# junwenxiong/diff_sal

Measured on AMD Instinct MI355X. Metric: denoise-steps/sec (batch x NFE / wall time), 16x224x384 clip, 50-step DPM-Solver, higher is better.
Workload: dtype f32; 1 GPU; BASELINE configs[1]: DHF1k visual-only, batch=4/GPU, 224x384, 50-NFE DPM-Solver (multistep-2, logSNR, denoise-to-zero), faithful full graph; batch_per_gpu=4, nfe_per_trajectory=50, step=one SalUNet evaluation + DPM-Solver update on one batch, sampler_mode=eager

## Files before the change

diff_sal_amd/_lib.py:

```python
import ctypes as C
import os

from . import build as _build

_LIB = None

c_f = C.c_void_p
c_i = C.c_int
c_fl = C.c_float
c_sz = C.c_size_t


class ConvDesc(C.Structure):

    _fields_ = [(n, C.c_int) for n in (
        "N", "H", "W", "Cin", "Ho", "Wo", "Cout", "KH", "KW", "stride_h", "stride_w", "pad_t", "pad_l",
        "dil_h", "dil_w", "act", "rowvec_ld", "w_format", "precision", "dtype")]


class Wino4Ext(C.Structure):

    _fields_ = [("in_ab", C.c_void_p), ("side_a", C.c_void_p), ("side_w", C.c_void_p), ("side_out", C.c_void_p),
                ("out_stats", C.c_void_p), ("up2_c", C.c_void_p), ("up2_scale", C.c_void_p), ("up2_shift", C.c_void_p),
                ("side_rows", C.c_longlong), ("in_swish", C.c_int), ("out_groups", C.c_int), ("up2_act", C.c_int), ("reserved", C.c_int)]


ABI_VERSION = 43


SIGNATURES = {
    "diffsal_version": (c_i, []),
    "diffsal_last_error": (C.c_char_p, []),
    "diffsal_last_gemm_kernel": (C.c_char_p, []),
    "diffsal_conv_igemm_group": (c_i, [c_i, c_f, c_f, c_f, c_f, c_f, c_f, c_sz, c_f]),
    "diffsal_kv_prep_proj": (c_i, [c_f] * 14 + [c_i, c_i, c_i, c_i, c_i, c_fl, c_f, c_f, c_fl, c_i, c_i, c_f]),
    "diffsal_block_front": (c_i, [c_f, c_f, c_f, c_f, c_f, c_fl, c_f, c_f, c_f, c_fl, c_f, c_f, c_f, c_f, c_f, c_i, c_i, c_i, c_i,
                                  c_i, c_i, c_fl, c_i, c_f]),
    "diffsal_set_tuning": (c_i, [C.c_char_p, c_i]),
    "diffsal_get_tuning": (c_i, [C.c_char_p]),
    "diffsal_temb_mlp": (c_i, [c_f, c_i, c_i, c_i, c_f, c_f, c_f, c_f, c_f, c_f, c_f, c_f]),
    "diffsal_dense_small": (c_i, [c_f, c_i, c_i, c_i, c_f, c_f, c_i, c_f, c_f]),
    "diffsal_conv_in": (c_i, [c_f, c_f, c_f, c_f, c_i, c_i, c_i, c_i, c_i, c_i, c_i, c_f]),
    "diffsal_maxpool2d": (c_i, [c_f, c_f, c_i, c_i, c_i, c_i, c_i, c_i, c_i, c_f]),
    "diffsal_conv_in_s4": (c_i, [c_f, c_f, c_f, c_f, c_i, c_i, c_i, c_i, c_i, c_f]),
    "diffsal_tapsum": (c_i, [c_f, c_f, c_f, c_i, c_f, c_i, c_i, c_i, c_i, c_i, c_f, c_f, c_f, c_i, c_i, c_f]),
    "diffsal_tapsum_head": (c_i, [c_f, c_f, c_f, c_i, c_i, c_i, c_i, c_i, c_i, c_f, c_f, c_f, c_i, c_f, c_f, c_f, c_i, c_f]),
    "diffsal_tapsum_bwd_ws_bytes": (C.c_long, [c_i, c_i, c_i, c_i]),
    "diffsal_tapsum_bwd": (c_i, [c_f, c_f, c_f, c_i, c_i, c_i, c_i, c_i, c_i, c_i, c_f]),
    "diffsal_groupnorm_ws_bytes": (c_sz, [c_i, c_i]),
    "diffsal_groupnorm_swish": (c_i, [c_f, c_f, c_f, c_f, c_i, c_i, c_i, c_i, c_fl, c_f, c_sz, c_i, c_f]),
    "diffsal_groupnorm": (c_i, [c_f, c_f, c_f, c_f, c_i, c_i, c_i, c_i, c_fl, c_i, c_f, c_sz, c_i, c_f]),
    "diffsal_softmax_rows": (c_i, [c_f, c_f, C.c_long, c_i, c_fl, c_f]),
# ... 176 lines not shown
```

diff_sal_amd/csrc/common.h:

```cpp
#pragma once
#include <hip/hip_runtime.h>

#include <cstdarg>
#include <cstdint>
#include <cstdio>

#include "../../include/diffsal.h"

namespace diffsal {

void set_error(const char* fmt, ...);
void note_kernel(const char* fmt, ...);

inline bool aligned16(const void* p) { return (reinterpret_cast<uintptr_t>(p) & 15u) == 0; }

inline int check_launch(const char* what) {
  hipError_t e = hipGetLastError();
  if (e != hipSuccess) {
    set_error("%s: launch failed: %s", what, hipGetErrorString(e));
    return DIFFSAL_E_LAUNCH;
  }
  return DIFFSAL_OK;
}

#define DS_REQUIRE(cond, code, ...)  \
  do {                               \
    if (!(cond)) {                   \
      diffsal::set_error(__VA_ARGS__); \
      return (code);                 \
    }                                \
  } while (0)

constexpr int kWave = 64;

enum TuneKey {
  TUNE_NO_PERSIST = 0, TUNE_NO_XCD_ORDER, TUNE_NO_HALO, TUNE_FORCE_HALO, TUNE_IGEMM_CFG, TUNE_IGEMM16_CFG, TUNE_PLAN_DEBUG,
  TUNE_WGRAD_CFG, TUNE_WGRAD_SPLITS, TUNE_WGRAD_VERBOSE, TUNE_NO_FUSED_BLOCK, TUNE_NO_WINOGRAD, TUNE_FORCE_WINOGRAD, TUNE_GN_CHUNKS,
  TUNE_GN_APPLY_WGS, TUNE_GEMM_DMA, TUNE_CONV_DMA, TUNE_GROUP_GRID, TUNE_GEMM_DMA16, TUNE_WGRAD_DMA, TUNE_NO_GN_SLAB, TUNE_NO_WINOGRAD4, TUNE_BATCH_TILE, TUNE_BATCH_XCD, TUNE_NO_TAPSUM_ROWS, TUNE_TAPSUM_ROWS_FORM,
  TUNE_NO_ATTN_BWD_DS, TUNE_NO_POOL_RUNS, TUNE_NO_ATTN_SLOTS, TUNE_NO_STREAM16, TUNE_CONV16_TILE, TUNE_BLOCK16_WAVES, TUNE_NO_ATTN16_MFMA, TUNE_CONV16_HALF, TUNE_COUNT
};
int tune(int key);

template <int CTRL>
__device__ __forceinline__ float dpp_move(float v) {
  return __builtin_bit_cast(float, __builtin_amdgcn_update_dpp(0, __builtin_bit_cast(int, v), CTRL, 0xF, 0xF, false));
}
__device__ __forceinline__ float lane_xor16(float v) {
  const unsigned u = __builtin_bit_cast(unsigned, v);
  const auto r = __builtin_amdgcn_permlane16_swap(u, u, false, false);
  return __builtin_bit_cast(float, (__lane_id() & 16) ? r[0] : r[1]);
}
__device__ __forceinline__ float lane_xor32(float v) {
  const unsigned u = __builtin_bit_cast(unsigned, v);
  const auto r = __builtin_amdgcn_permlane32_swap(u, u, false, false);
// ... 290 lines not shown
```

diff_sal_amd/csrc/misc.hip:

```cpp
#include "common.h"

#include <cstdlib>
#include <cstring>

namespace diffsal {

static thread_local char g_err[512] = "";
void set_error(const char* fmt, ...) {
  va_list ap;
  va_start(ap, fmt);
  vsnprintf(g_err, sizeof(g_err), fmt, ap);
  va_end(ap);
}

static thread_local char g_kernel[160] = "";
void note_kernel(const char* fmt, ...) {
  va_list ap;
  va_start(ap, fmt);
  vsnprintf(g_kernel, sizeof(g_kernel), fmt, ap);
  va_end(ap);
}

static const char* const kTuneNames[TUNE_COUNT] = {
    "DIFFSAL_NO_PERSIST", "DIFFSAL_NO_XCD_ORDER", "DIFFSAL_NO_HALO", "DIFFSAL_FORCE_HALO", "DIFFSAL_IGEMM_CFG",
    "DIFFSAL_IGEMM16_CFG", "DIFFSAL_PLAN_DEBUG", "DIFFSAL_WGRAD_CFG", "DIFFSAL_WGRAD_SPLITS", "DIFFSAL_WGRAD_VERBOSE",
    "DIFFSAL_NO_FUSED_BLOCK", "DIFFSAL_NO_WINOGRAD", "DIFFSAL_FORCE_WINOGRAD", "DIFFSAL_GN_CHUNKS", "DIFFSAL_GN_APPLY_WGS",
    "DIFFSAL_GEMM_DMA", "DIFFSAL_CONV_DMA", "DIFFSAL_GROUP_GRID", "DIFFSAL_GEMM_DMA16", "DIFFSAL_WGRAD_DMA", "DIFFSAL_NO_GN_SLAB", "DIFFSAL_NO_WINOGRAD4", "DIFFSAL_BATCH_TILE", "DIFFSAL_BATCH_XCD", "DIFFSAL_NO_TAPSUM_ROWS", "DIFFSAL_TAPSUM_ROWS_FORM",
    "DIFFSAL_NO_ATTN_BWD_DS", "DIFFSAL_NO_POOL_RUNS", "DIFFSAL_NO_ATTN_SLOTS", "DIFFSAL_NO_STREAM16", "DIFFSAL_CONV16_TILE", "DIFFSAL_BLOCK16_WAVES", "DIFFSAL_NO_ATTN16_MFMA", "DIFFSAL_CONV16_HALF"};
static int g_tune[TUNE_COUNT];
static const bool g_tune_init = [] {
  for (int k = 0; k < TUNE_COUNT; ++k) {
    const char* e = getenv(kTuneNames[k]);
    g_tune[k] = (e && e[0]) ? atoi(e) : -1;
  }
  return true;
}();
int tune(int key) { return (key >= 0 && key < TUNE_COUNT) ? __atomic_load_n(&g_tune[key], __ATOMIC_RELAXED) : -1; }

__global__ __launch_bounds__(256) void temb_dense0_kernel(const void* __restrict__ t, int t_is_f32, int B, int ch,
                                                          const float* __restrict__ freq, const float* __restrict__ w0,
                                                          const float* __restrict__ b0, float* __restrict__ hid) {
  extern __shared__ float sh[];
  const int half = ch / 2, tc = 4 * ch;
// ... 849 lines not shown
    case DIFFSAL_WS_CONV_WINO4_STATS: return d && have && n_dims == 1 ? diffsal_conv_wino4_stats_bytes(d, D(0)) : 0;
    case DIFFSAL_WS_CONV_WGRAD: return d ? diffsal_conv_wgrad_ws_bytes(d) : 0;
    case DIFFSAL_WS_WGRAD_SEGMENTED: return have && n_dims == 4 ? diffsal_wgrad_segmented_ws_bytes(D(0), D(1), D(2), D(3)) : 0;
    case DIFFSAL_WS_TAPSUM_BWD: return have && n_dims == 4 ? static_cast<size_t>(diffsal_tapsum_bwd_ws_bytes(D(0), D(1), D(2), D(3))) : 0;
    case DIFFSAL_WS_SALIENCY_METRICS: return have && n_dims == 1 ? diffsal_saliency_metrics_ws_bytes(D(0)) : 0;
    case DIFFSAL_WS_ATTENTION_TAIL:
      return have && n_dims == 5 ? sizeof(float) * diffsal_attention_general_tail_floats(D(0), D(1), D(2), D(3), D(4)) : 0;
    case DIFFSAL_WS_ATTENTION_BWD_QTAIL:
      return have && n_dims == 6 ? sizeof(float) * diffsal_attention_general_bwd_qtail_floats(D(0), D(1), D(2), D(3), D(4), D(5)) : 0;
    case DIFFSAL_WS_ATTENTION_BWD_DS:
      return have && n_dims == 4 ? sizeof(float) * diffsal_attention_general_bwd_ds_floats(D(0), D(1), D(2), D(3)) : 0;
    default: return 0;
  }
}

extern "C" int diffsal_version(void) { return 43; }
extern "C" const char* diffsal_last_error(void) { return g_err; }
extern "C" const char* diffsal_last_gemm_kernel(void) { return g_kernel; }

extern "C" int diffsal_set_tuning(const char* name, int value) {
  DS_REQUIRE(name, DIFFSAL_E_ARG, "set_tuning: null name");
  for (int k = 0; k < TUNE_COUNT; ++k)
    if (strcmp(name, kTuneNames[k]) == 0) {
      __atomic_store_n(&g_tune[k], value, __ATOMIC_RELAXED);
      return DIFFSAL_OK;
    }
  set_error("set_tuning: unknown switch '%s'", name);
  return DIFFSAL_E_ARG;
}
extern "C" int diffsal_get_tuning(const char* name) {
  if (name)
// ... 550 lines not shown
```

diff_sal_amd/csrc/tblock.hip:

```cpp
#include "common.h"

namespace diffsal {

template <> struct Mfma32x16<float> { typedef f32x8_t vec; };

template <typename T>
struct FrontArgs {
  const T* x;
  const T* k;
  const T* v;
  const float* g1; const float* b1;
  const float* w9;
  const float* gq; const float* bq;
  const T* wq; const float* bias_q;
  const T* wp; const float* bias_p;
  T* out;
  int N, H, W, Lk;
  float eps1, epsq, scale;
  int tiles_y, tiles_x;
#ifdef DIFFSAL_DEV_STAMPS
  unsigned long long* stamps;
#endif
};

// ... 487 lines not shown
template <typename T, int C>
static int launch_front(const FrontArgs<T>& a, hipStream_t s) {
  typedef FrontLds<T, C> L;
  DS_RAISE_DYNAMIC_LDS((block_front_kernel<T, C>), 160 * 1024);
  const int n_tiles = a.N * a.tiles_y * a.tiles_x;
  const int resident = 256 * (L::total * 2 <= 160 * 1024 ? 2 : 1);
  const int grid = n_tiles < resident ? n_tiles : resident;
#ifdef DIFFSAL_DEV_STAMPS
  FrontArgs<T> b = a;
  b.stamps = (g_front_stamps && static_cast<size_t>(grid) * 64 * 8 <= g_front_stamp_bytes) ? g_front_stamps : nullptr;
  hipLaunchKernelGGL((block_front_kernel<T, C>), dim3(grid), dim3(256), L::total, s, b);
  return check_launch("block_front");
#endif
  hipLaunchKernelGGL((block_front_kernel<T, C>), dim3(grid), dim3(256), L::total, s, a);
  return check_launch("block_front");
}

}

using namespace diffsal;

#ifdef DIFFSAL_DEV_STAMPS
extern "C" int diffsal_set_front_stamps(void* device_buffer, size_t bytes) {
  diffsal::g_front_stamps = static_cast<unsigned long long*>(device_buffer);
  diffsal::g_front_stamp_bytes = device_buffer ? bytes : 0;
  return DIFFSAL_OK;
}
#endif

extern "C" int diffsal_block_front(const void* x, const void* k, const void* v, const float* g1, const float* b1, float eps1,
// ... 18 lines not shown
  {                                                                                                                         \
    FrontArgs<T> a{static_cast<const T*>(x), static_cast<const T*>(k), static_cast<const T*>(v), g1, b1, w9, gq, bq,        \
                   static_cast<const T*>(wq), bias_q, static_cast<const T*>(wp), bias_p, static_cast<T*>(out), N, H, W, Lk, \
                   eps1, epsq, scale, tiles_y, tiles_x};                                                                    \
    return launch_front<T, CC>(a, s);                                                                                       \
  }
  if (dtype == DIFFSAL_F32) DS_FRONT(float, 96)
  if (C == 96) {
    if (dtype == DIFFSAL_BF16) DS_FRONT(bf16_t, 96)
    DS_FRONT(f16_t, 96)
  }
  if (dtype == DIFFSAL_BF16) DS_FRONT(bf16_t, 192)
  DS_FRONT(f16_t, 192)
#undef DS_FRONT
}
```

diff_sal_amd/ops.py:

```python
from __future__ import annotations

import contextlib
import ctypes as C
import threading
from typing import List, Optional, Sequence, Tuple

import torch

from . import _lib
from ._lib import ACT_GELU, ACT_GELU_GRAD, ACT_NONE, ACT_RELU, ACT_SIGMOID, ConvDesc

Tensor = torch.Tensor

PROFILE = None


_PROF_DEPTH = [0]


class _prof:
    __slots__ = ("cls", "flops", "nbytes", "e0", "note", "counted", "kernel")

    def __init__(self, cls, flops=0.0, nbytes=0.0, note="", kernel=""):
        self.cls, self.flops, self.nbytes, self.e0, self.note, self.counted = cls, float(flops), float(nbytes), None, note, False
# ... 965 lines not shown
    with_p = x.dtype == torch.float32
    if with_p and lin_p is None:
        raise RuntimeError("block_front: fp32 storage needs the output projection")
    M = N * H * W
    fl = 2.0 * M * Cc * Cc * (2 if with_p else 1) + 4.0 * M * Lk * Cc + 22.0 * M * Cc
    with _prof("K10f", fl, _nb(x, out, k, v, lin_q[0]) + (_nb(lin_p[0]) if with_p else 0.0), f"block_front M={M} C={Cc}",
               kernel=f"block_front_kernel<{'float' if with_p else '16-bit'}, {Cc}>"):
        _lib.check(lib.diffsal_block_front(_pa(x, dt), _pa(k, dt), _pa(v, dt), _p(norm1[0]), _p(norm1[1]), float(norm1[2]),
                                           _p(w9), _p(norm_q[0]), _p(norm_q[1]), float(norm_q[2]), _pa(lin_q[0], dt),
                                           _p(lin_q[1]), _pa(lin_p[0], dt) if with_p else None,
                                           _p(lin_p[1]) if with_p else None, out.data_ptr(), N, H, W, Cc, Lk, heads,
                                           float(scale), dt, _stream()), "block_front")
    return out


def dwpool_ln_kv(xk: Tensor, xv: Tensor, wk: Tensor, wv: Tensor, gk: Tensor, bk: Tensor, gv: Tensor, bv: Tensor,
                 k: int, eps: float = 1e-5):
    lib = _lib.load()
    N, H, W, Cc = xv.shape
    gh, gw = (H - k) // k + 1, (W - k) // k + 1
    ok = torch.empty((N, gh * gw, Cc), device=xv.device, dtype=xv.dtype)
    ov = torch.empty_like(ok)
    dt = _dt(xv)
    with _prof("K9", 4.0 * N * H * W * Cc, _nb(xk, ok, ov) + (0.0 if xk.data_ptr() == xv.data_ptr() else _nb(xv))):
        _lib.check(lib.diffsal_dwpool_ln_kv(_pa(xk, dt), _pa(xv, dt), _p(wk), _p(wv), _p(gk), _p(bk), _p(gv), _p(bv),
                                            ok.data_ptr(), ov.data_ptr(), N, H, W, Cc, k, eps, dt, _stream()), "dwpool_ln_kv")
    return ok, ov


def attention(q: Tensor, k: Tensor, v: Tensor, heads: int, scale: float) -> Tensor:
# ... 890 lines not shown
```

diff_sal_amd/sal_unet.py:

```python
from __future__ import annotations

import math
from typing import Dict, List, Optional, Sequence

import torch
from torch import nn

from . import ops
from .ops import ACT_GELU, ACT_NONE, ACT_RELU

Tensor = torch.Tensor


def _holder(**children) -> nn.Module:
    m = nn.Module()
    for k, v in children.items():
        setattr(m, k, v)
    return m


def _seq_named(pairs) -> nn.Sequential:
    from collections import OrderedDict

    return nn.Sequential(OrderedDict(pairs))
# ... 163 lines not shown
                if m.bias is not None:
                    nn.init.zeros_(m.bias)
            elif isinstance(m, (nn.LayerNorm, nn.BatchNorm2d, nn.GroupNorm)):
                nn.init.ones_(m.weight)
                nn.init.zeros_(m.bias)
        for st in self.invpt_decoder.mid_stages:
            for m in st.modules():
                if isinstance(m, nn.Linear):
                    nn.init.trunc_normal_(m.weight, std=0.02)
        nn.init.trunc_normal_(self.invpt_decoder.mt_proj[0].weight, std=0.02)

    def _precision(self) -> str:
        return self.gemm_precision or ops.get_gemm_precision()

    def _cache_key(self):
        return (self._pack_epoch, self._precision(), self.compute_dtype, self.winograd, self.fold_attn_proj) + tuple(
            (p.data_ptr(), p._version) for p in list(self.parameters()) + list(self.buffers()))

    def pack_epoch(self):
        return self._cache_key()

    def parameters_updated(self) -> None:
        self._pack_epoch += 1

    def _pack_conv(self, w: Tensor) -> Tensor:
        wp = ops.pack_conv_weight(w)
        if self.compute_dtype != torch.float32:
            return ops.cast(wp, self.compute_dtype)
        return ops.split_weight(wp) if self._precision() == "bf16x3" else wp

    def _pack_wino(self, w: Tensor, f2: bool = True):
# ... 8 lines not shown
    def _use_tap_conv(self, taps, which: str) -> bool:
        if not self.tap_conv or (taps is not None and self.taps_reference_forms):
            return False
        if (which == "mt" and self.compute_dtype != torch.float32 and self.mt_tap16_f32 and self.fold_head
                and self.ori_embed_dim % 192 == 0):
            return True
        return self.compute_dtype == torch.float32 or which in self.tap_conv16

    def _gemm_w(self, w: Tensor) -> Tensor:
        return w.detach() if self.compute_dtype == torch.float32 else ops.cast(w.detach().contiguous(), self.compute_dtype)

    def _fold_attn(self, i: int, Lk: int) -> bool:
        return (self.fold_attn_proj and self.compute_dtype == torch.float32 and self._precision() == "fp32"
                and ops.attn_fold_supported(self.up_channels[i], self.heads[i], Lk, torch.float32))

    @staticmethod
    def fold_attn_weights(a: nn.Module):
        c = a.proj_q.weight.shape[0]
        d = c // 2
        wq, wk, wv, wp = (l.weight.detach().double() for l in (a.proj_q, a.proj_k, a.proj_v, a.proj))
        zero = wq.new_zeros(c)
        bq, bv, bp = ((l.bias.detach().double() if l.bias is not None else zero) for l in (a.proj_q, a.proj_v, a.proj))
        kq, vp, ukq = [], [], []
        for h in range(2):
            s = slice(h * d, (h + 1) * d)
            kq.append(wq[s].t() @ wk[s])
            vp.append(wp[:, s] @ wv[s])
            ukq.append(wk[s].t() @ bq[s])
        return (torch.cat(kq, 0).float().contiguous(), torch.cat(vp, 0).float().contiguous(),
                torch.stack(ukq, 0).float().contiguous(), (bp + wp @ bv).float().contiguous())

    @staticmethod
    def _bn_affine(bn: nn.BatchNorm2d):
        scale = (bn.weight.detach() / torch.sqrt(bn.running_var + bn.eps)).contiguous()
        shift = (bn.bias.detach() - bn.running_mean * scale).contiguous()
        return scale, shift

    def packed(self) -> Dict[str, Tensor]:
        key = self._cache_key()
        if self._pack_cache is not None and key == self._pack_key:
            return self._pack_cache
        dev = self.conv_in.weight.device
        pk: Dict[str, Tensor] = {}
        half = self.ch // 2
        pk["freq"] = torch.exp(torch.arange(half, dtype=torch.float32) * -(math.log(10000) / (half - 1))).to(dev)
# ... 28 lines not shown
                pk[f"s{i}.pe2.w"] = self._pack_conv(pe[4].weight)
                pk[f"s{i}.pe2.wino"] = self._pack_wino(pe[4].weight)
                pk[f"s{i}.pe2.scale"], pk[f"s{i}.pe2.shift"] = self._bn_affine(pe[5])
            a = st.blocks[0].attn
            c = self.up_channels[i]
            k = self.kernel_kv[i]
            pk[f"s{i}.wq9"] = a.conv_proj_q.conv.weight.detach()[:, 0, 1].reshape(c, 9).t().contiguous()
            pk[f"s{i}.wk"] = a.conv_proj_k.conv.weight.detach().reshape(c, k * k).t().contiguous()
            pk[f"s{i}.wv"] = a.conv_proj_v.conv.weight.detach().reshape(c, k * k).t().contiguous()
            pk[f"s{i}.align.w"] = self._gemm_w(st.blocks[0].align_conv.weight.detach().reshape(c, 512).contiguous())
            blk = st.blocks[0]
            for nm, lin in (("q", a.proj_q), ("k", a.proj_k), ("v", a.proj_v), ("proj", a.proj), ("fc1", blk.mlp.fc1),
                            ("fc2", blk.mlp.fc2)):
                pk[f"s{i}.{nm}.w"] = self._gemm_w(lin.weight)
            pk[f"s{i}.redu.w"] = self._pack_conv(dec.redu_chan_up[i].proj[0].weight)
            if self._fold_attn(i, 1):
                pk[f"s{i}.kq.w"], pk[f"s{i}.vp.w"], pk[f"s{i}.ukq"], pk[f"s{i}.proj.bf"] = self.fold_attn_weights(a)
        if all(f"s{i}.align.w" in pk for i in range(self.num_stages)) and self.num_stages > 1:
            pk["align_all.w"] = torch.cat([pk[f"s{i}.align.w"] for i in range(self.num_stages)], 0).contiguous()
            pk["align_all.b"] = torch.cat([dec.mid_stages[i].blocks[0].align_conv.bias.detach().float()
                                           for i in range(self.num_stages)], 0).contiguous()
            offs, o = [], 0
            for i in range(self.num_stages):
                offs.append(o)
                o += self.up_channels[i]
            pk["align_all.offs"] = offs
        pk["mt.w"] = self._pack_conv(dec.mt_proj[0].weight)
        pk["mt.tapw"] = self._tap_weight(dec.mt_proj[0].weight)
        pk["mt.scale"], pk["mt.shift"] = self._bn_affine(dec.mt_proj[1])
        pk["head.w"] = self.logits.linear_pred.weight.detach().reshape(-1).contiguous()
        self._pack_cache, self._pack_key = pk, key
# ... 74 lines not shown
            if isinstance(audio_tok, tuple):
                a_all, offs = audio_tok
                a_small = a_all[:, :, offs[i]:offs[i] + C]
            else:
                a_small = ops.linear(audio_tok, pk[f"s{i}.align.w"], blk.align_conv.bias, tag="K7-align")
            k_src = ops.audio_fuse(a_small, x, audio_hw[0], audio_hw[1])
        xt = x.view(n9, H * W, C)
        gh, gw = (H - self.kernel_kv[i]) // self.kernel_kv[i] + 1, (W - self.kernel_kv[i]) // self.kernel_kv[i] + 1
        if (self.fused_front and ops.block_front_supported(C, self.heads[i], gh * gw, x.dtype)
                and (x.dtype != torch.float32 or self._precision() == "fp32")
                and not getattr(pk[f"s{i}.k.w"], "_diffsal_split", False)):
            xv_ = x.view(n9, H, W, C)
            xk_ = xv_ if k_src is None else k_src.view(n9, H, W, C)
            kvn = (a.conv_proj_k.bn.weight, a.conv_proj_k.bn.bias, a.conv_proj_v.bn.weight, a.conv_proj_v.bn.bias)
            pre = (blk.norm.weight, blk.norm.bias, blk.norm.eps, k_src is None)
            if self.fold_kv_proj and C == 96:
                kk, vv = ops.kv_prep_proj(xk_, xv_, pk[f"s{i}.wk"], pk[f"s{i}.wv"], *kvn, self.kernel_kv[i], a.conv_proj_k.bn.eps, pre,
                                          (pk[f"s{i}.k.w"], a.proj_k.bias), (pk[f"s{i}.v.w"], a.proj_v.bias))
            else:
                kk, vv = ops.kv_prep(xk_, xv_, pk[f"s{i}.wk"], pk[f"s{i}.wv"], *kvn, self.kernel_kv[i], a.conv_proj_k.bn.eps, pre_ln=pre)
                kk, vv = ops.linear_pair(kk, vv, pk[f"s{i}.k.w"], pk[f"s{i}.v.w"], a.proj_k.bias, a.proj_v.bias)
            f32 = x.dtype == torch.float32
            y = ops.block_front(xv_, kk, vv, (blk.norm.weight, blk.norm.bias, blk.norm.eps), pk[f"s{i}.wq9"],
                                (a.conv_proj_q.bn.weight, a.conv_proj_q.bn.bias, a.conv_proj_q.bn.eps),
                                (pk[f"s{i}.q.w"], a.proj_q.bias), (pk[f"s{i}.proj.w"], a.proj.bias) if f32 else None,
                                self.heads[i], float(C) ** -0.5).view(n9, H * W, C)
            nz = None if norm_z is None else (norm_z.weight, norm_z.bias, norm_z.eps)
            if C == 96 and blk.mlp.fc1.out_features == 192:
                if f32:
                    x2, z = ops.mlp_block(y, (blk.norm2.weight, blk.norm2.bias, blk.norm2.eps), (pk[f"s{i}.fc1.w"], blk.mlp.fc1.bias),
                                          (pk[f"s{i}.fc2.w"], blk.mlp.fc2.bias), nz, (H * W, T, self.temporal_list[i]))
                else:
                    x2, z = ops.block16(y, xt, (pk[f"s{i}.proj.w"], a.proj.bias), (blk.norm2.weight, blk.norm2.bias, blk.norm2.eps),
                                        (pk[f"s{i}.fc1.w"], blk.mlp.fc1.bias), (pk[f"s{i}.fc2.w"], blk.mlp.fc2.bias), nz,
                                        (H * W, T, self.temporal_list[i]))
                return x2.view(B, T, H, W, C), (None if z is None else z.view(B, T, H, W, C))
            x1 = y if f32 else ops.linear(y, pk[f"s{i}.proj.w"], a.proj.bias, residual=xt)
            y2 = ops.layernorm(x1, blk.norm2.weight, blk.norm2.bias, blk.norm2.eps)
            y2 = ops.linear(y2, pk[f"s{i}.fc1.w"], blk.mlp.fc1.bias, act=ACT_GELU)
            x2 = ops.linear(y2, pk[f"s{i}.fc2.w"], blk.mlp.fc2.bias, residual=x1)
            return x2.view(B, T, H, W, C), None
# ... 73 lines not shown
                    per_clip.append(T * h * w * 9 * self.up_channels[i])
                h, w = 2 * h, 2 * w
            per_clip.append(T * h * w * self.up_channels[i] * 2)
            tok += h * w
        per_clip.append(tok * 9 * self.down_channel * (2 if es == 2 else 1) if tap_form else 4 * h * w * self.ori_embed_dim)
        worst = max(per_clip)
        by_bytes = ((1 << 32) - (1 << 24)) // (worst * es)
        by_count = ((1 << 31) - (1 << 24)) // worst
        return max(1, min(self.max_clips_per_pass, by_bytes, by_count))

    tap_conv = True
    fold_norm1 = False
    fused_front = True
    fold_kv_proj = False
    fold_attn_proj = True
    winograd = True
    fuse_resblock = True
    taps_reference_forms = False
    _freq_tables: dict = {}
    fold_head = True
    merge_qkv_prep = True
    pair_kv = True
    up_commute = True
    up_commute16 = True
    fuse_up_pe2 = True
    group_qkv = True
    group_qkv_all = False
    merge_align = True
    group_reduce_temp = True
    tap_conv16 = ()
# ... 369 lines not shown
```

include/diffsal.h:

```cpp
#ifndef DIFFSAL_H
#define DIFFSAL_H

#include <stddef.h>
#include <stdint.h>

#ifdef __cplusplus
extern "C" {
#endif

typedef void* diffsal_stream_t;

enum {
  DIFFSAL_OK = 0,
  DIFFSAL_E_SHAPE = -1,
  DIFFSAL_E_ALIGN = -2,
  DIFFSAL_E_LAUNCH = -3,
  DIFFSAL_E_ARG = -4
};

enum { DIFFSAL_ACT_NONE = 0, DIFFSAL_ACT_RELU = 1, DIFFSAL_ACT_GELU_ERF = 2, DIFFSAL_ACT_SIGMOID = 3,
       DIFFSAL_ACT_GELU_GRAD = 5 };

int diffsal_version(void);
const char* diffsal_last_error(void);
// ... 249 lines not shown
                      diffsal_stream_t stream);

int diffsal_head_sigmoid(const void* x, const float* w , const float* bias , float* out ,
                         int NHW, int C, int dtype, diffsal_stream_t stream);

int diffsal_kv_prep_proj(const void* xk, const void* xv, const float* wk, const float* wv, const float* gk, const float* bk,
                         const float* gv, const float* bv, const void* proj_wk, const float* proj_bk, const void* proj_wv,
                         const float* proj_bv, void* out_k, void* out_v, int N, int H, int W, int C, int k, float eps,
                         const float* pre_gamma, const float* pre_beta, float pre_eps, int pre_ln_k, int dtype,
                         diffsal_stream_t stream);

int diffsal_block_front(const void* x, const void* k, const void* v, const float* g1, const float* b1, float eps1,
                        const float* w9, const float* gq, const float* bq, float epsq, const void* wq, const float* bias_q,
                        const void* wp, const float* bias_p, void* out, int N, int H, int W, int C, int Lk, int heads,
                        float scale, int dtype, diffsal_stream_t stream);

int diffsal_cast(const void* src, int src_dtype, void* dst, int dst_dtype, long n, diffsal_stream_t stream);

int diffsal_attention_general(const float* q, const float* q_extra, const float* k, const float* k_extra,
                              const int* k_slots , const float* v, const float* residual, float* out, float* lse , int B,
                              int H, int Lq, int Lk, int D, int E, int DV, const long* q_strides ,
                              const long* k_strides, const long* v_strides, const long* r_strides, float scale,
                              int skip_first, float* tail_ws, size_t tail_ws_floats, diffsal_stream_t stream);
size_t diffsal_attention_general_tail_floats(int B, int H, int Lq, int Lk, int DV);
int diffsal_attention_general_bwd_splits(int B, int H, int Lq, int Lk);
size_t diffsal_attention_general_bwd_qtail_floats(int B, int H, int Lq, int Lk, int D, int E);
size_t diffsal_attention_general_bwd_ds_floats(int B, int H, int Lq, int Lk);
int diffsal_attention_general_bwd(const float* q, const float* q_extra, const float* k, const float* k_extra, const float* v,
                                  const float* residual, const float* out, const float* lse, const float* dout,
                                  float* delta_ws, float* kv_part_ws, float* q_tail_ws, size_t q_tail_ws_floats, float* ds_ws,
// ... 84 lines not shown
```

Baseline: 1239 denoise-steps/s.

## Add folded-projection block front kernel that absorbs q/k/v/proj weights into attention

Adds a new fused block-front kernel for C=96, 2-head, f32 stages. It uses precomputed folded matrices (Wq^T Wk and Wp Wv per head) so attention scores and outputs come straight from the normalized depthwise-conv query and small per-key matrices. This removes the separate q projection GEMM and output projection GEMM per token, moving work onto the few keys instead. The folded weights change rounding slightly and add a separate kv_prep plus linear_pair path for G and U.

```diff
diff --git a/diff_sal_amd/_lib.py b/diff_sal_amd/_lib.py
--- a/diff_sal_amd/_lib.py
+++ b/diff_sal_amd/_lib.py
@@ -25,7 +25,7 @@
                 ("side_rows", C.c_longlong), ("in_swish", C.c_int), ("out_groups", C.c_int), ("up2_act", C.c_int), ("reserved", C.c_int)]
 
 
-ABI_VERSION = 43
+ABI_VERSION = 44
 
 
 SIGNATURES = {
@@ -36,6 +36,7 @@
     "diffsal_kv_prep_proj": (c_i, [c_f] * 14 + [c_i, c_i, c_i, c_i, c_i, c_fl, c_f, c_f, c_fl, c_i, c_i, c_f]),
     "diffsal_block_front": (c_i, [c_f, c_f, c_f, c_f, c_f, c_fl, c_f, c_f, c_f, c_fl, c_f, c_f, c_f, c_f, c_f, c_i, c_i, c_i, c_i,
                                   c_i, c_i, c_fl, c_i, c_f]),
+    "diffsal_block_front_fold": (c_i, [c_f] * 7 + [c_fl] + [c_f] * 3 + [c_fl, c_f, c_f] + [c_i] * 6 + [c_fl, c_f]),
     "diffsal_set_tuning": (c_i, [C.c_char_p, c_i]),
     "diffsal_get_tuning": (c_i, [C.c_char_p]),
     "diffsal_temb_mlp": (c_i, [c_f, c_i, c_i, c_i, c_f, c_f, c_f, c_f, c_f, c_f, c_f, c_f]),
diff --git a/diff_sal_amd/csrc/common.h b/diff_sal_amd/csrc/common.h
--- a/diff_sal_amd/csrc/common.h
+++ b/diff_sal_amd/csrc/common.h
@@ -37,7 +37,7 @@
   TUNE_NO_PERSIST = 0, TUNE_NO_XCD_ORDER, TUNE_NO_HALO, TUNE_FORCE_HALO, TUNE_IGEMM_CFG, TUNE_IGEMM16_CFG, TUNE_PLAN_DEBUG,
   TUNE_WGRAD_CFG, TUNE_WGRAD_SPLITS, TUNE_WGRAD_VERBOSE, TUNE_NO_FUSED_BLOCK, TUNE_NO_WINOGRAD, TUNE_FORCE_WINOGRAD, TUNE_GN_CHUNKS,
   TUNE_GN_APPLY_WGS, TUNE_GEMM_DMA, TUNE_CONV_DMA, TUNE_GROUP_GRID, TUNE_GEMM_DMA16, TUNE_WGRAD_DMA, TUNE_NO_GN_SLAB, TUNE_NO_WINOGRAD4, TUNE_BATCH_TILE, TUNE_BATCH_XCD, TUNE_NO_TAPSUM_ROWS, TUNE_TAPSUM_ROWS_FORM,
-  TUNE_NO_ATTN_BWD_DS, TUNE_NO_POOL_RUNS, TUNE_NO_ATTN_SLOTS, TUNE_NO_STREAM16, TUNE_CONV16_TILE, TUNE_BLOCK16_WAVES, TUNE_NO_ATTN16_MFMA, TUNE_CONV16_HALF, TUNE_COUNT
+  TUNE_NO_ATTN_BWD_DS, TUNE_NO_POOL_RUNS, TUNE_NO_ATTN_SLOTS, TUNE_NO_STREAM16, TUNE_CONV16_TILE, TUNE_BLOCK16_WAVES, TUNE_NO_ATTN16_MFMA, TUNE_CONV16_HALF, TUNE_FRONT_FOLD_WGS, TUNE_COUNT
 };
 int tune(int key);
 
diff --git a/diff_sal_amd/csrc/misc.hip b/diff_sal_amd/csrc/misc.hip
--- a/diff_sal_amd/csrc/misc.hip
+++ b/diff_sal_amd/csrc/misc.hip
@@ -26,7 +26,7 @@
     "DIFFSAL_IGEMM16_CFG", "DIFFSAL_PLAN_DEBUG", "DIFFSAL_WGRAD_CFG", "DIFFSAL_WGRAD_SPLITS", "DIFFSAL_WGRAD_VERBOSE",
     "DIFFSAL_NO_FUSED_BLOCK", "DIFFSAL_NO_WINOGRAD", "DIFFSAL_FORCE_WINOGRAD", "DIFFSAL_GN_CHUNKS", "DIFFSAL_GN_APPLY_WGS",
     "DIFFSAL_GEMM_DMA", "DIFFSAL_CONV_DMA", "DIFFSAL_GROUP_GRID", "DIFFSAL_GEMM_DMA16", "DIFFSAL_WGRAD_DMA", "DIFFSAL_NO_GN_SLAB", "DIFFSAL_NO_WINOGRAD4", "DIFFSAL_BATCH_TILE", "DIFFSAL_BATCH_XCD", "DIFFSAL_NO_TAPSUM_ROWS", "DIFFSAL_TAPSUM_ROWS_FORM",
-    "DIFFSAL_NO_ATTN_BWD_DS", "DIFFSAL_NO_POOL_RUNS", "DIFFSAL_NO_ATTN_SLOTS", "DIFFSAL_NO_STREAM16", "DIFFSAL_CONV16_TILE", "DIFFSAL_BLOCK16_WAVES", "DIFFSAL_NO_ATTN16_MFMA", "DIFFSAL_CONV16_HALF"};
+    "DIFFSAL_NO_ATTN_BWD_DS", "DIFFSAL_NO_POOL_RUNS", "DIFFSAL_NO_ATTN_SLOTS", "DIFFSAL_NO_STREAM16", "DIFFSAL_CONV16_TILE", "DIFFSAL_BLOCK16_WAVES", "DIFFSAL_NO_ATTN16_MFMA", "DIFFSAL_CONV16_HALF", "DIFFSAL_FRONT_FOLD_WGS"};
 static int g_tune[TUNE_COUNT];
 static const bool g_tune_init = [] {
   for (int k = 0; k < TUNE_COUNT; ++k) {
@@ -906,7 +906,7 @@
   }
 }
 
-extern "C" int diffsal_version(void) { return 43; }
+extern "C" int diffsal_version(void) { return 44; }
 extern "C" const char* diffsal_last_error(void) { return g_err; }
 extern "C" const char* diffsal_last_gemm_kernel(void) { return g_kernel; }
 
diff --git a/diff_sal_amd/csrc/tblock.hip b/diff_sal_amd/csrc/tblock.hip
--- a/diff_sal_amd/csrc/tblock.hip
+++ b/diff_sal_amd/csrc/tblock.hip
@@ -525,6 +525,368 @@
 #endif
   hipLaunchKernelGGL((block_front_kernel<T, C>), dim3(grid), dim3(256), L::total, s, a);
   return check_launch("block_front");
+}
+
+
+struct FrontFoldArgs {
+  const float* x;
+  const float* G;
+  const float* U;
+  const float* kp;
+  const float* ukq;
+  const float* g1; const float* b1;
+  const float* w9;
+  const float* gq; const float* bq;
+  const float* bias;
+  float* out;
+  int N, H, W, Lk;
+  float eps1, epsq, scale;
+  int tiles_y, tiles_x;
+#ifdef DIFFSAL_DEV_STAMPS
+  unsigned long long* stamps;
+#endif
+};
+
+struct FrontFoldLds {
+  static constexpr int C = 96;
+  static constexpr int PW = C + 4;
+  static constexpr int PU = 68;
+  static constexpr int vec_floats = 9 * C + 3 * C + 2 * C + 2 * C + 64;
+  static constexpr size_t vec_bytes = static_cast<size_t>(vec_floats) * sizeof(float);
+  static constexpr size_t tile_bytes = static_cast<size_t>(FT_TOK) * PW * sizeof(float);
+  static constexpr size_t gu_bytes = (static_cast<size_t>(64) * PW + static_cast<size_t>(C) * PU) * sizeof(float);
+  static constexpr size_t region_bytes = ((tile_bytes > gu_bytes ? tile_bytes : gu_bytes) + 15) / 16 * 16;
+  static constexpr size_t total = vec_bytes + region_bytes;
+};
+static_assert(2 * FrontFoldLds::total <= 160 * 1024, "two workgroups of the folded front share a CU's LDS");
+
+template <bool AHEAD>
+__global__ __launch_bounds__(256, (AHEAD ? 1 : 2)) void block_front_fold_kernel(FrontFoldArgs p) {
+#pragma clang fp contract(off)
+  typedef FrontFoldLds L;
+  constexpr int C = L::C, PW = L::PW, PX = L::PW, PU = L::PU;
+  constexpr int NU = C / 32, NG = C / 8, HEADS = 2, NP = C / 4, G = NP / 3;
+
+  extern __shared__ __attribute__((aligned(16))) unsigned char smraw[];
+  float* vecs = reinterpret_cast<float*>(smraw);
+  float* ukqs = vecs + 12 * C;
+  float* ln1s = vecs + 14 * C;
+  float* s0s = vecs + 16 * C;
+  float* region = reinterpret_cast<float*>(smraw + L::vec_bytes);
+  float* xns = region;
+  float* Gs = region;
+  float* Uts = region + 64 * PW;
+
+  const int tid = threadIdx.x, lane = tid & 63, wave = tid >> 6;
+  const int ml = lane & 31, hf = lane >> 5;
+
+  for (int i = tid; i < 9 * C; i += 256) vecs[i] = p.w9[i];
+  for (int i = tid; i < C; i += 256) {
+    vecs[9 * C + i] = p.gq[i]; vecs[10 * C + i] = p.bq[i]; vecs[11 * C + i] = p.bias[i];
+    ukqs[i] = p.ukq[i]; ukqs[C + i] = p.ukq[C + i];
+    ln1s[i] = p.g1[i]; ln1s[C + i] = p.b1[i];
+  }
+  const int a_slot = tid / G, a_sub = tid - a_slot * G;
+  float4 ga[3], ba[3];
+  if constexpr (AHEAD) {
+#pragma unroll
+    for (int i = 0; i < 3; ++i) { ga[i] = ld4(p.g1 + 4 * (a_sub + G * i)); ba[i] = ld4(p.b1 + 4 * (a_sub + G * i)); }
+  }
+  __syncthreads();
+
+  const int n_tiles = p.N * p.tiles_y * p.tiles_x;
+  const int trow = 2 * wave + (ml >> 4), tcol = ml & 15;
+  const int centre = (trow + 1) * FT_HW + (tcol + 1);
+  const float* gf = Gs + ml * PW + 4 * hf;
+  const float* uf = Uts + ml * PU + 4 * hf;
+
+  auto opaque = [](int v) { asm volatile("" : "+v"(v)); return v; };
+
+  constexpr int TPP = 256 / G;
+  constexpr int NPASS = (FT_TOK + TPP - 1) / TPP;
+  float4 pre[NPASS][3];
+  unsigned inside_mask = 0;
+  auto fetch_tile = [&](int tile_) -> unsigned {
+    const int tx_ = tile_ % p.tiles_x, t2_ = tile_ / p.tiles_x;
+    const int ty_ = t2_ % p.tiles_y, n_ = t2_ / p.tiles_y;
+    const float* ximg_ = p.x + static_cast<long>(n_) * p.H * p.W * C;
+    unsigned mask = 0;
+    const int t_ = opaque(tid), slot_ = t_ / G, sub_ = t_ - slot_ * G;
+#pragma unroll
+    for (int ps = 0; ps < NPASS; ++ps) {
+      const int tok = ps * TPP + slot_;
+      const int hy = tok / FT_HW, hx = tok - hy * FT_HW;
+      const int gy = ty_ * FT_TH + hy - 1, gx = tx_ * FT_TW + hx - 1;
+      const bool inside = tok < FT_TOK && gy >= 0 && gy < p.H && gx >= 0 && gx < p.W;
+      const float* src = ximg_ + (static_cast<long>(inside ? gy : 0) * p.W + (inside ? gx : 0)) * C;
+#pragma unroll
+      for (int i = 0; i < 3; ++i) pre[ps][i] = ld4(src + 4 * (sub_ + G * i));
+      mask |= (inside ? 1u : 0u) << ps;
+    }
+    return mask;
+  };
+  const bool xcd_walk = (n_tiles & 7) == 0 && (gridDim.x & 7) == 0;
+  auto tile_of = [&](int v) { return xcd_walk ? (v & 7) * (n_tiles >> 3) + (v >> 3) : v; };
+  if (AHEAD && static_cast<int>(blockIdx.x) < n_tiles) inside_mask = fetch_tile(tile_of(blockIdx.x));
+
+#ifdef DIFFSAL_DEV_STAMPS
+  int stamp_it = 0;
+  auto stamp = [&](int k) {
+    if (p.stamps && tid == 0 && stamp_it < 8) p.stamps[(static_cast<long>(blockIdx.x) * 8 + stamp_it) * 8 + k] = wall_clock64();
+  };
+#else
+  auto stamp = [](int) {};
+#endif
+  for (int vt = blockIdx.x; vt < n_tiles; vt += gridDim.x) {
+    const int tile = tile_of(vt);
+    stamp(0);
+    const int tx = tile % p.tiles_x, t2 = tile / p.tiles_x;
+    const int ty = t2 % p.tiles_y, n = t2 / p.tiles_y;
+    const int y0 = ty * FT_TH, x0 = tx * FT_TW;
+    if constexpr (!AHEAD) inside_mask = fetch_tile(tile);
+
+#pragma unroll
+    for (int ps = 0; ps < NPASS; ++ps) {
+      const int tok = ps * TPP + a_slot;
+      const bool inside = (inside_mask >> ps) & 1u;
+      float4 vv[3];
+#pragma unroll
+      for (int i = 0; i < 3; ++i) vv[i] = pre[ps][i];
+      float s = 0.f;
+#pragma unroll
+      for (int i = 0; i < 3; ++i) s += (vv[i].x + vv[i].y) + (vv[i].z + vv[i].w);
+      s = group_sum<G>(s);
+      const float mean = s * (1.0f / C);
+      float qq = 0.f;
+#pragma unroll
+      for (int i = 0; i < 3; ++i) {
+        const float a = vv[i].x - mean, b = vv[i].y - mean, c = vv[i].z - mean, d = vv[i].w - mean;
+        qq += (a * a + b * b) + (c * c + d * d);
+      }
+      qq = group_sum<G>(qq);
+      const float rstd = 1.0f / sqrtf(qq * (1.0f / C) + p.eps1);
+      if (tok < FT_TOK) {
+#pragma unroll
+        for (int i = 0; i < 3; ++i) {
+          if constexpr (!AHEAD) { ga[i] = ld4(ln1s + 4 * (a_sub + G * i)); ba[i] = ld4(ln1s + C + 4 * (a_sub + G * i)); }
+          float4 o;
+          o.x = inside ? (vv[i].x - mean) * rstd * ga[i].x + ba[i].x : 0.f;
+          o.y = inside ? (vv[i].y - mean) * rstd * ga[i].y + ba[i].y : 0.f;
+          o.z = inside ? (vv[i].z - mean) * rstd * ga[i].z + ba[i].z : 0.f;
+          o.w = inside ? (vv[i].w - mean) * rstd * ga[i].w + ba[i].w : 0.f;
+          st4(xns + tok * PX + 4 * (a_sub + G * i), o);
+        }
+      }
+    }
+    __syncthreads();
+    stamp(1);
+    constexpr int NGP = 64 * NP / 256;
+    float4 graw[NGP], uraw[NGP], kraw[3];
+    auto fetch_u = [&]() {
+      const float* usrc = p.U + static_cast<long>(n) * p.Lk * 2 * C;
+      const int t_ = opaque(tid);
+#pragma unroll
+      for (int i = 0; i < NGP; ++i) {
+        const int pc = t_ + 256 * i;
+        const int ru = pc & 63, ju = ru & 31;
+        uraw[i] = ld4(usrc + (ju < p.Lk ? ju : 0) * 2 * C + (ru >> 5) * C + 4 * (pc >> 6));
+      }
+    };
+    {
+      const float* gsrc = p.G + static_cast<long>(n) * p.Lk * 2 * C;
+      const int t_ = opaque(tid);
+#pragma unroll
+      for (int i = 0; i < NGP; ++i) {
+        const int pc = t_ + 256 * i;
+        const int rg = pc / NP, jg = rg & 31;
+        graw[i] = ld4(gsrc + (jg < p.Lk ? jg : 0) * 2 * C + (rg >> 5) * C + 4 * (pc - rg * NP));
+      }
+      const int key = t_ >> 3;
+#pragma unroll
+      for (int i = 0; i < 3; ++i)
+        kraw[i] = ld4(p.kp + (static_cast<long>(n) * p.Lk + (key < p.Lk ? key : 0)) * C + 4 * ((t_ & 7) + 8 * i));
+    }
+    if constexpr (AHEAD) fetch_u();
+
+    float4 qin[NG];
+#pragma unroll
+    for (int g = 0; g < NG; ++g) qin[g] = make_float4(0.f, 0.f, 0.f, 0.f);
+    {
+      constexpr int HG = 6, SPT = NG / HG, NSTEP = 9 * SPT;
+      float4 xa[2][HG], wa[2][HG];
+      auto issue = [&](int step, float4 (&xd)[HG], float4 (&wd)[HG]) {
+        const int tap = step / SPT, g0 = (step % SPT) * HG;
+        const int off = (tap / 3 - 1) * FT_HW + (tap % 3 - 1);
+        const float* xs = xns + (centre + off) * PX + 4 * hf + 8 * g0;
+        const float* ws = vecs + tap * C + 4 * hf + 8 * g0;
+#pragma unroll
+        for (int g = 0; g < HG; ++g) { xd[g] = ld4(xs + 8 * g); wd[g] = ld4(ws + 8 * g); }
+      };
+      issue(0, xa[0], wa[0]);
+#pragma unroll
+      for (int step = 0; step < NSTEP; ++step) {
+        if (step + 1 < NSTEP) issue(step + 1, xa[(step + 1) & 1], wa[(step + 1) & 1]);
+        __builtin_amdgcn_sched_barrier(0);
+        const int g0 = (step % SPT) * HG;
+#pragma unroll
+        for (int g = 0; g < HG; ++g) {
+          const float4 a = xa[step & 1][g], w = wa[step & 1][g];
+          qin[g0 + g].x = fmaf(a.x, w.x, qin[g0 + g].x); qin[g0 + g].y = fmaf(a.y, w.y, qin[g0 + g].y);
+          qin[g0 + g].z = fmaf(a.z, w.z, qin[g0 + g].z); qin[g0 + g].w = fmaf(a.w, w.w, qin[g0 + g].w);
+        }
+        __builtin_amdgcn_sched_barrier(0);
+      }
+    }
+    if constexpr (!AHEAD) fetch_u();
+    {
+      float s = 0.f;
+#pragma unroll
+      for (int g = 0; g < NG; ++g) s += (qin[g].x + qin[g].y) + (qin[g].z + qin[g].w);
+      s += lane_xor32(s);
+      const float mean = s * (1.0f / C);
+      float qq = 0.f;
+#pragma unroll
+      for (int g = 0; g < NG; ++g) {
+        const float a = qin[g].x - mean, b = qin[g].y - mean, c = qin[g].z - mean, d = qin[g].w - mean;
+        qq += (a * a + b * b) + (c * c + d * d);
+      }
+      qq += lane_xor32(qq);
+      const float rstd = 1.0f / sqrtf(qq * (1.0f / C) + p.epsq);
+#pragma unroll
+      for (int g = 0; g < NG; ++g) {
+        const float4 gm = ld4(vecs + 9 * C + 8 * g + 4 * hf), bt = ld4(vecs + 10 * C + 8 * g + 4 * hf);
+        qin[g].x = (qin[g].x - mean) * rstd * gm.x + bt.x; qin[g].y = (qin[g].y - mean) * rstd * gm.y + bt.y;
+        qin[g].z = (qin[g].z - mean) * rstd * gm.z + bt.z; qin[g].w = (qin[g].w - mean) * rstd * gm.w + bt.w;
+      }
+    }
+    __syncthreads();
+    stamp(2);
+
+    const int tc = opaque(tid);
+#pragma unroll
+    for (int i = 0; i < NGP; ++i) {
+      const int pc = tc + 256 * i;
+      const int rg = pc / NP;
+      st4(Gs + rg * PW + 4 * (pc - rg * NP), (rg & 31) < p.Lk ? graw[i] : make_float4(0.f, 0.f, 0.f, 0.f));
+      const int ru = pc & 63, c4 = 4 * (pc >> 6);
+      const bool oku = (ru & 31) < p.Lk;
+      Uts[(c4 + 0) * PU + ru] = oku ? uraw[i].x : 0.f;
+      Uts[(c4 + 1) * PU + ru] = oku ? uraw[i].y : 0.f;
+      Uts[(c4 + 2) * PU + ru] = oku ? uraw[i].z : 0.f;
+      Uts[(c4 + 3) * PU + ru] = oku ? uraw[i].w : 0.f;
+    }
+    {
+      float d0 = 0.f, d1 = 0.f;
+#pragma unroll
+      for (int i = 0; i < 3; ++i) {
+        const float4 u0 = ld4(ukqs + 4 * ((tc & 7) + 8 * i)), u1 = ld4(ukqs + C + 4 * ((tc & 7) + 8 * i));
+        d0 = fmaf(kraw[i].x, u0.x, d0); d0 = fmaf(kraw[i].y, u0.y, d0); d0 = fmaf(kraw[i].z, u0.z, d0); d0 = fmaf(kraw[i].w, u0.w, d0);
+        d1 = fmaf(kraw[i].x, u1.x, d1); d1 = fmaf(kraw[i].y, u1.y, d1); d1 = fmaf(kraw[i].z, u1.z, d1); d1 = fmaf(kraw[i].w, u1.w, d1);
+      }
+      d0 = group_sum<8>(d0);
+      d1 = group_sum<8>(d1);
+      const int key = tc >> 3;
+      if ((tc & 7) == 0) {
+        s0s[key] = key < p.Lk ? d0 : 0.f;
+        s0s[32 + key] = key < p.Lk ? d1 : 0.f;
+      }
+    }
+    __syncthreads();
+    stamp(3);
+    if (AHEAD && vt + static_cast<int>(gridDim.x) < n_tiles) inside_mask = fetch_tile(tile_of(vt + gridDim.x));
+
+    const int gy = y0 + trow, gx = x0 + tcol;
+    const bool live = gy < p.H && gx < p.W;
+    const long tokoff = ((static_cast<long>(n) * p.H + (live ? gy : 0)) * p.W + (live ? gx : 0)) * C + 4 * hf;
+    float4 xres[NU * 4];
+#pragma unroll
+    for (int i = 0; i < NU * 4; ++i) xres[i] = ld4(p.x + tokoff + 8 * i);
+
+    f32x16 pt[HEADS];
+#pragma unroll
+    for (int hd = 0; hd < HEADS; ++hd) {
+      f32x16 st;
+#pragma unroll
+      for (int g = 0; g < 4; ++g) {
+        const float4 s4 = ld4(s0s + 32 * hd + 8 * g + 4 * hf);
+        st[4 * g + 0] = s4.x; st[4 * g + 1] = s4.y; st[4 * g + 2] = s4.z; st[4 * g + 3] = s4.w;
+      }
+      mfma_groups_f32<NG>([&](int i) { return gf + 32 * hd * PW + 8 * i; },
+                          [&](int i, float4 a) { DS_MFMA4(st, a, qin[i].x, qin[i].y, qin[i].z, qin[i].w); });
+      float mx = -3.0e38f;
+#pragma unroll
+      for (int r = 0; r < 16; ++r) {
+        const bool ok = (r & 3) + 8 * (r >> 2) + 4 * hf < p.Lk;
+        mx = ok ? fmaxf(mx, st[r]) : mx;
+      }
+      mx = fmaxf(mx, lane_xor32(mx));
+      float sum = 0.f;
+#pragma unroll
+      for (int r = 0; r < 16; ++r) {
+        const bool ok = (r & 3) + 8 * (r >> 2) + 4 * hf < p.Lk;
+        const float e = ok ? __expf((st[r] - mx) * p.scale) : 0.f;
+        st[r] = e;
+        sum += e;
+      }
+      sum += lane_xor32(sum);
+      const float inv = 1.0f / sum;
+#pragma unroll
+      for (int r = 0; r < 16; ++r) pt[hd][r] = st[r] * inv;
+    }
+
+    stamp(4);
+    f32x16 x1[NU];
+#pragma unroll
+    for (int t = 0; t < NU; ++t)
+#pragma unroll
+      for (int g = 0; g < 4; ++g) {
+        const float4 b4 = ld4(vecs + 11 * C + 32 * t + 8 * g + 4 * hf);
+        x1[t][4 * g + 0] = b4.x; x1[t][4 * g + 1] = b4.y; x1[t][4 * g + 2] = b4.z; x1[t][4 * g + 3] = b4.w;
+      }
+#pragma unroll
+    for (int g = 0; g < 4; ++g) {
+      if (8 * g < p.Lk) {
+        mfma_groups_f32<HEADS * NU>([&](int i) { return uf + 32 * (i % NU) * PU + 32 * (i / NU) + 8 * g; },
+                                    [&](int i, float4 a) {
+                                      const int t = i % NU, hd = i / NU;
+                                      DS_MFMA4(x1[t], a, pt[hd][4 * g + 0], pt[hd][4 * g + 1], pt[hd][4 * g + 2], pt[hd][4 * g + 3]);
+                                    });
+      }
+    }
+    if (live) {
+      float* dst = p.out + tokoff;
+#pragma unroll
+      for (int t = 0; t < NU; ++t)
+#pragma unroll
+        for (int g = 0; g < 4; ++g) {
+          const float4 r4 = xres[4 * t + g];
+          st4(dst + 32 * t + 8 * g, make_float4(x1[t][4 * g + 0] + r4.x, x1[t][4 * g + 1] + r4.y, x1[t][4 * g + 2] + r4.z,
+                                                x1[t][4 * g + 3] + r4.w));
+        }
+    }
+    __syncthreads();
+    stamp(5);
+#ifdef DIFFSAL_DEV_STAMPS
+    ++stamp_it;
+#endif
+  }
+}
+
+template <bool AHEAD>
+static int launch_front_fold(const FrontFoldArgs& a, hipStream_t s) {
+  typedef FrontFoldLds L;
+  DS_RAISE_DYNAMIC_LDS((block_front_fold_kernel<AHEAD>), 160 * 1024);
+  const int n_tiles = a.N * a.tiles_y * a.tiles_x;
+  const int resident = 256 * (AHEAD ? 1 : 2);
+  const int grid = n_tiles < resident ? n_tiles : resident;
+#ifdef DIFFSAL_DEV_STAMPS
+  FrontFoldArgs b = a;
+  b.stamps = (g_front_stamps && static_cast<size_t>(grid) * 64 * 8 <= g_front_stamp_bytes) ? g_front_stamps : nullptr;
+  hipLaunchKernelGGL((block_front_fold_kernel<AHEAD>), dim3(grid), dim3(256), L::total, s, b);
+#else
+  hipLaunchKernelGGL((block_front_fold_kernel<AHEAD>), dim3(grid), dim3(256), L::total, s, a);
+#endif
+  return check_launch("block_front_fold");
 }
 
 }
@@ -573,3 +935,22 @@
   DS_FRONT(f16_t, 192)
 #undef DS_FRONT
 }
+
+extern "C" int diffsal_block_front_fold(const float* x, const float* G, const float* U, const float* kp, const float* ukq,
+                                        const float* g1, const float* b1, float eps1, const float* w9, const float* gq,
+                                        const float* bq, float epsq, const float* bias, float* out, int N, int H, int W, int C,
+                                        int Lk, int heads, float scale, diffsal_stream_t stream) {
+  DS_REQUIRE(x && G && U && kp && ukq && g1 && b1 && w9 && gq && bq && bias && out, DIFFSAL_E_ARG, "block_front_fold: null argument");
+  DS_REQUIRE(C == 96 && heads == 2, DIFFSAL_E_SHAPE, "block_front_fold: built for C = 96, 2 heads (got C = %d, %d heads)", C, heads);
+  DS_REQUIRE(N > 0 && H > 0 && W > 0 && Lk > 0 && Lk <= 32, DIFFSAL_E_SHAPE, "block_front_fold: N=%d H=%d W=%d Lk=%d (Lk <= 32)", N, H, W, Lk);
+  DS_REQUIRE(static_cast<long>(N) * H * W * C < (1L << 31), DIFFSAL_E_SHAPE, "block_front_fold: tensor too large for one launch");
+  DS_REQUIRE(aligned16(x) && aligned16(out) && aligned16(G) && aligned16(U) && aligned16(kp) && aligned16(ukq) && aligned16(g1) &&
+                 aligned16(b1) && aligned16(w9) && aligned16(gq) && aligned16(bq) && aligned16(bias),
+             DIFFSAL_E_ALIGN, "block_front_fold: misaligned pointer (every operand is read in 16-byte pieces)");
+  DS_REQUIRE(out != x, DIFFSAL_E_ARG, "block_front_fold: in-place operation is not supported (neighbouring tiles read the halo)");
+  FrontFoldArgs a{x, G, U, kp, ukq, g1, b1, w9, gq, bq, bias, out, N, H, W, Lk, eps1, epsq, scale,
+                  (H + FT_TH - 1) / FT_TH, (W + FT_TW - 1) / FT_TW};
+  hipStream_t s = static_cast<hipStream_t>(stream);
+  if (tune(TUNE_FRONT_FOLD_WGS) == 1) return launch_front_fold<true>(a, s);
+  return launch_front_fold<false>(a, s);
+}
diff --git a/diff_sal_amd/ops.py b/diff_sal_amd/ops.py
--- a/diff_sal_amd/ops.py
+++ b/diff_sal_amd/ops.py
@@ -1003,6 +1003,29 @@
     return out
 
 
+def block_front_fold_supported(C: int, heads: int, Lk: int, dtype: torch.dtype = torch.float32) -> bool:
+    return dtype == torch.float32 and heads == 2 and 0 < Lk <= 32 and C == 96
+
+
+def block_front_fold(x: Tensor, G: Tensor, U: Tensor, kp: Tensor, ukq: Tensor, norm1, w9: Tensor, norm_q, bias: Tensor, heads: int,
+                     scale: float) -> Tensor:
+    lib = _lib.load()
+    N, H, W, Cc = x.shape
+    Lk = kp.shape[1]
+    if (x.dtype != torch.float32 or G.shape != (N, Lk, heads * Cc) or U.shape != G.shape or kp.shape != (N, Lk, Cc)
+            or ukq.shape != (heads, Cc) or bias.shape != (Cc,)):
+        raise RuntimeError(f"block_front_fold: inconsistent shapes x {tuple(x.shape)} G {tuple(G.shape)} U {tuple(U.shape)} "
+                           f"kp {tuple(kp.shape)} ukq {tuple(ukq.shape)} bias {tuple(bias.shape)}")
+    out = torch.empty_like(x)
+    M = N * H * W
+    fl = 2.0 * M * Cc * 64 + 2.0 * M * Cc * heads * (-(-Lk // 8) * 8) + 22.0 * M * Cc
+    with _prof("K10f", fl, _nb(x, out, G, U, kp), f"block_front_fold M={M} C={Cc}", kernel="block_front_fold_kernel"):
+        _lib.check(lib.diffsal_block_front_fold(_p(x), _p(G), _p(U), _p(kp), _p(ukq), _p(norm1[0]), _p(norm1[1]), float(norm1[2]),
+                                                _p(w9), _p(norm_q[0]), _p(norm_q[1]), float(norm_q[2]), _p(bias), _p(out), N, H, W,
+                                                Cc, Lk, heads, float(scale), _stream()), "block_front_fold")
+    return out
+
+
 def dwpool_ln_kv(xk: Tensor, xv: Tensor, wk: Tensor, wv: Tensor, gk: Tensor, bk: Tensor, gv: Tensor, bv: Tensor,
                  k: int, eps: float = 1e-5):
     lib = _lib.load()
diff --git a/diff_sal_amd/sal_unet.py b/diff_sal_amd/sal_unet.py
--- a/diff_sal_amd/sal_unet.py
+++ b/diff_sal_amd/sal_unet.py
@@ -201,7 +201,7 @@
         return self.gemm_precision or ops.get_gemm_precision()
 
     def _cache_key(self):
-        return (self._pack_epoch, self._precision(), self.compute_dtype, self.winograd, self.fold_attn_proj) + tuple(
+        return (self._pack_epoch, self._precision(), self.compute_dtype, self.winograd, self.fold_attn_proj, self.fold_front_proj, self.fused_front) + tuple(
             (p.data_ptr(), p._version) for p in list(self.parameters()) + list(self.buffers()))
 
     def pack_epoch(self):
@@ -240,8 +240,12 @@
         return (self.fold_attn_proj and self.compute_dtype == torch.float32 and self._precision() == "fp32"
                 and ops.attn_fold_supported(self.up_channels[i], self.heads[i], Lk, torch.float32))
 
+    def _fold_front(self, i: int, Lk: int) -> bool:
+        return (self.fold_front_proj and self.fused_front and self.compute_dtype == torch.float32 and self._precision() == "fp32"
+                and ops.block_front_fold_supported(self.up_channels[i], self.heads[i], Lk, torch.float32))
+
     @staticmethod
-    def fold_attn_weights(a: nn.Module):
+    def fold_attn_weights(a: nn.Module, dtype: torch.dtype = torch.float32):
         c = a.proj_q.weight.shape[0]
         d = c // 2
         wq, wk, wv, wp = (l.weight.detach().double() for l in (a.proj_q, a.proj_k, a.proj_v, a.proj))
@@ -253,8 +257,7 @@
             kq.append(wq[s].t() @ wk[s])
             vp.append(wp[:, s] @ wv[s])
             ukq.append(wk[s].t() @ bq[s])
-        return (torch.cat(kq, 0).float().contiguous(), torch.cat(vp, 0).float().contiguous(),
-                torch.stack(ukq, 0).float().contiguous(), (bp + wp @ bv).float().contiguous())
+        return tuple(t.to(dtype).contiguous() for t in (torch.cat(kq, 0), torch.cat(vp, 0), torch.stack(ukq, 0), bp + wp @ bv))
 
     @staticmethod
     def _bn_affine(bn: nn.BatchNorm2d):
@@ -313,7 +316,7 @@
                             ("fc2", blk.mlp.fc2)):
                 pk[f"s{i}.{nm}.w"] = self._gemm_w(lin.weight)
             pk[f"s{i}.redu.w"] = self._pack_conv(dec.redu_chan_up[i].proj[0].weight)
-            if self._fold_attn(i, 1):
+            if self._fold_attn(i, 1) or self._fold_front(i, 1):
                 pk[f"s{i}.kq.w"], pk[f"s{i}.vp.w"], pk[f"s{i}.ukq"], pk[f"s{i}.proj.bf"] = self.fold_attn_weights(a)
         if all(f"s{i}.align.w" in pk for i in range(self.num_stages)) and self.num_stages > 1:
             pk["align_all.w"] = torch.cat([pk[f"s{i}.align.w"] for i in range(self.num_stages)], 0).contiguous()
@@ -418,17 +421,25 @@
             xk_ = xv_ if k_src is None else k_src.view(n9, H, W, C)
             kvn = (a.conv_proj_k.bn.weight, a.conv_proj_k.bn.bias, a.conv_proj_v.bn.weight, a.conv_proj_v.bn.bias)
             pre = (blk.norm.weight, blk.norm.bias, blk.norm.eps, k_src is None)
-            if self.fold_kv_proj and C == 96:
+            f32 = x.dtype == torch.float32
+            fold = f32 and self._fold_front(i, gh * gw)
+            if fold:
+                kk, vv = ops.kv_prep(xk_, xv_, pk[f"s{i}.wk"], pk[f"s{i}.wv"], *kvn, self.kernel_kv[i], a.conv_proj_k.bn.eps, pre_ln=pre)
+                Gk, Uv = ops.linear_pair(kk, vv, pk[f"s{i}.kq.w"], pk[f"s{i}.vp.w"], None, None)
+                y = ops.block_front_fold(xv_, Gk, Uv, kk, pk[f"s{i}.ukq"], (blk.norm.weight, blk.norm.bias, blk.norm.eps),
+                                         pk[f"s{i}.wq9"], (a.conv_proj_q.bn.weight, a.conv_proj_q.bn.bias, a.conv_proj_q.bn.eps),
+                                         pk[f"s{i}.proj.bf"], self.heads[i], float(C) ** -0.5).view(n9, H * W, C)
+            elif self.fold_kv_proj and C == 96:
                 kk, vv = ops.kv_prep_proj(xk_, xv_, pk[f"s{i}.wk"], pk[f"s{i}.wv"], *kvn, self.kernel_kv[i], a.conv_proj_k.bn.eps, pre,
                                           (pk[f"s{i}.k.w"], a.proj_k.bias), (pk[f"s{i}.v.w"], a.proj_v.bias))
             else:
                 kk, vv = ops.kv_prep(xk_, xv_, pk[f"s{i}.wk"], pk[f"s{i}.wv"], *kvn, self.kernel_kv[i], a.conv_proj_k.bn.eps, pre_ln=pre)
                 kk, vv = ops.linear_pair(kk, vv, pk[f"s{i}.k.w"], pk[f"s{i}.v.w"], a.proj_k.bias, a.proj_v.bias)
-            f32 = x.dtype == torch.float32
-            y = ops.block_front(xv_, kk, vv, (blk.norm.weight, blk.norm.bias, blk.norm.eps), pk[f"s{i}.wq9"],
-                                (a.conv_proj_q.bn.weight, a.conv_proj_q.bn.bias, a.conv_proj_q.bn.eps),
-                                (pk[f"s{i}.q.w"], a.proj_q.bias), (pk[f"s{i}.proj.w"], a.proj.bias) if f32 else None,
-                                self.heads[i], float(C) ** -0.5).view(n9, H * W, C)
+            if not fold:
+                y = ops.block_front(xv_, kk, vv, (blk.norm.weight, blk.norm.bias, blk.norm.eps), pk[f"s{i}.wq9"],
+                                    (a.conv_proj_q.bn.weight, a.conv_proj_q.bn.bias, a.conv_proj_q.bn.eps),
+                                    (pk[f"s{i}.q.w"], a.proj_q.bias), (pk[f"s{i}.proj.w"], a.proj.bias) if f32 else None,
+                                    self.heads[i], float(C) ** -0.5).view(n9, H * W, C)
             nz = None if norm_z is None else (norm_z.weight, norm_z.bias, norm_z.eps)
             if C == 96 and blk.mlp.fc1.out_features == 192:
                 if f32:
@@ -532,6 +543,7 @@
     fused_front = True
     fold_kv_proj = False
     fold_attn_proj = True
+    fold_front_proj = True
     winograd = True
     fuse_resblock = True
     taps_reference_forms = False
diff --git a/include/diffsal.h b/include/diffsal.h
--- a/include/diffsal.h
+++ b/include/diffsal.h
@@ -287,6 +287,11 @@
                         const float* w9, const float* gq, const float* bq, float epsq, const void* wq, const float* bias_q,
                         const void* wp, const float* bias_p, void* out, int N, int H, int W, int C, int Lk, int heads,
                         float scale, int dtype, diffsal_stream_t stream);
+
+int diffsal_block_front_fold(const float* x, const float* G, const float* U, const float* kp, const float* ukq, const float* g1,
+                             const float* b1, float eps1, const float* w9, const float* gq, const float* bq, float epsq,
+                             const float* bias, float* out, int N, int H, int W, int C, int Lk, int heads, float scale,
+                             diffsal_stream_t stream);
 
 int diffsal_cast(const void* src, int src_dtype, void* dst, int dst_dtype, long n, diffsal_stream_t stream);
 
```

Result: faster. 1261 denoise-steps/s, median of 6 (+1.8%).
